# quokka-astro/quokka

Measured on AMD Instinct MI355X. Metric: Mcell-updates/s on 3D Sedov unigrid, higher is better.
Workload: dtype f64; 1 GPU; 3D Sedov blast 256x256x256 unigrid (tests/blast_unigrid_256.in scaled to 256^3 cells per GPU), 128^3 boxes, PPM+HLLC RK2, gamma=1.4, CFL 0.3, reflecting octant; cells_per_gpu=16777216, boxes_per_gpu=8, parallelism=box-decomposition x1, rk2_mode=carry, fofc_stages=0, retries=0, x_sweep_in_y_march=True

## Files before the change

### include/quokka_amd.h

```cpp
#ifndef QUOKKA_AMD_H_
#define QUOKKA_AMD_H_

#include <stdint.h>

#ifdef __cplusplus
extern "C" {
#endif

typedef struct qk_ctx qk_ctx;
typedef struct qk_level qk_level;
typedef void *qk_stream;

typedef enum qk_status {
	QK_OK = 0,
	QK_ERR_INVALID = -1,
	QK_ERR_HIP = -2,
	QK_ERR_UNSUPPORTED = -3,
	QK_ERR_STATE = -4
} qk_status;

typedef struct qk_array4 {
	double *p;
	int64_t jstride, kstride, nstride;
	int begin[3];
// ... 88 lines not shown
int qk_advect_ComputeFluxes(qk_level *lev, qk_stream s, int dir, qk_array4 *flux, const qk_array4 *left, const qk_array4 *right, double advectionVx, int nvars);
int qk_advect_PredictStep(qk_level *lev, qk_stream s, const qk_array4 *consVarOld, qk_array4 *consVarNew, const qk_array4 *const fluxArray[3], double dt,
			  const double dx[3], int nvars);
int qk_advect_AddFluxesRK2(qk_level *lev, qk_stream s, qk_array4 *U_new, const qk_array4 *U0, const qk_array4 *U1, const qk_array4 *const fluxArray[3], double dt,
			   const double dx[3], int nvars);

typedef struct qk_hydro_stage_args {
	const qk_array4 *U_in;
	const qk_array4 *U_old;
	qk_array4 *U_out;
	qk_array4 *halfFlux[3];
	qk_array4 *halfVel[3];
	qk_iarray4 *redoFlag;
	int64_t *d_redo_count;
	int *d_error_flag;
	double *d_max_signal;
	void *scratch;
	int64_t scratch_bytes;
	double dx[3];
	double dt;
	int stage;
	int reconstruction_order;
	double densityFloor, tempFloor;
	int use_dual_energy;
	double K_visc;
	int store_flux_rk2;
	qk_array4 *fluxRk2[3];
	int rk2_carry_rhs;
	qk_array4 *rhs1;
	const struct qk_carray4 *flux_mask;
	int fofc_pass;
	int prim_out;
	int prim_in;
} qk_hydro_stage_args;

int64_t qk_hydro_stage_scratch_bytes(qk_level *lev, const qk_hydro_traits *t);
int qk_hydro_stage_fused(qk_level *lev, qk_stream s, const qk_hydro_traits *t, const qk_hydro_stage_args *a);

#define QK_MAX_GROUPS 8
typedef struct qk_rad_traits {
	double c_light, c_hat, radiation_constant, Erad_floor;
	int beta_order;
	int opacity_model;
	double kappaP, kappaE, kappaF;
	int pow_mode;
	int eddington_model;
	double opacity_T_ref, opacity_T_exponent, opacity_pow_floor;
	int ngroups;
	int mg_opacity_model;
	double energy_unit;
	double rad_boundaries[QK_MAX_GROUPS + 1];
	double mg_kappa_exponent[QK_MAX_GROUPS + 1], mg_kappa_lower[QK_MAX_GROUPS + 1];
	double mg_kappa_rho_exponent, mg_kappa_T_ref, mg_kappa_T_exponent;
	int enable_dust_gas_thermal_coupling_model;
	double dust_gas_interaction_coeff;
	int thermal_model;
	double gas_dust_coupling_threshold;
	double cooling_linear_coeff[QK_MAX_GROUPS];
	double cr_heating_rate;
	int enable_photoelectric_heating;
	double pe_heating_E1_derivative;
} qk_rad_traits;

int qk_rad_ConservedToPrimitive(qk_level *lev, qk_stream s, const qk_rad_traits *rt, const qk_array4 *cons, qk_array4 *primVar, int nghost);
int qk_rad_ComputeWavespeedCorrection(qk_level *lev, qk_stream s, const qk_rad_traits *rt, const qk_hydro_traits *t, int ndim, const qk_array4 *consVar,
				      const double dx[3], qk_array4 *const eps[3]);
int qk_rad_ComputeFluxes(qk_level *lev, qk_stream s, const qk_rad_traits *rt, int dir, qk_array4 *x1Flux, const qk_array4 *x1LeftState,
			 const qk_array4 *x1RightState, const qk_array4 *consVar, const qk_array4 *wavespeed_eps);
// ... 169 lines not shown
```

### quokka_amd/capi.py

```python
from __future__ import annotations

import ctypes as C
import os

_HERE = os.path.dirname(os.path.abspath(__file__))
LIB_PATH = os.environ.get("QK_LIB_PATH", os.path.join(_HERE, "lib", "libquokka_amd.so"))

QK_OK, QK_ERR_INVALID, QK_ERR_HIP, QK_ERR_UNSUPPORTED, QK_ERR_STATE = 0, -1, -2, -3, -4
ERR_UNSUPPORTED = QK_ERR_UNSUPPORTED
HOOK_COMPILED = 100
DIR_X1, DIR_X2, DIR_X3 = 0, 1, 2
RIEMANN_HLLC, RIEMANN_LLF, RIEMANN_HLLD = 0, 1, 2
LIMITER_MINMOD, LIMITER_MC = 0, 1
BC_REFLECT_ODD, BC_INT_DIR, BC_REFLECT_EVEN, BC_FOEXTRAP, BC_EXT_DIR = -1, 0, 1, 2, 3

K_B = 1.380649e-16
M_U = 1.6605390666e-24


class Array4(C.Structure):
    _fields_ = [("p", C.c_void_p), ("jstride", C.c_int64), ("kstride", C.c_int64), ("nstride", C.c_int64),
                ("begin", C.c_int * 3), ("end", C.c_int * 3), ("ncomp", C.c_int)]


# ... 33 lines not shown
                ("ngroups", C.c_int), ("mg_opacity_model", C.c_int), ("energy_unit", C.c_double), ("rad_boundaries", C.c_double * (MAX_GROUPS + 1)),
                ("mg_kappa_exponent", C.c_double * (MAX_GROUPS + 1)), ("mg_kappa_lower", C.c_double * (MAX_GROUPS + 1)),
                ("mg_kappa_rho_exponent", C.c_double), ("mg_kappa_T_ref", C.c_double), ("mg_kappa_T_exponent", C.c_double),
                ("enable_dust_gas_thermal_coupling_model", C.c_int), ("dust_gas_interaction_coeff", C.c_double), ("thermal_model", C.c_int),
                ("gas_dust_coupling_threshold", C.c_double),
                ("cooling_linear_coeff", C.c_double * MAX_GROUPS), ("cr_heating_rate", C.c_double), ("enable_photoelectric_heating", C.c_int),
                ("pe_heating_E1_derivative", C.c_double)]

    def set_groups(self, boundaries, energy_unit, opacity_model, kappa_exponent, kappa_lower, rho_exponent=0.0, T_ref=0.0, T_exponent=0.0):
        ng = len(boundaries) - 1
        assert 2 <= ng <= MAX_GROUPS and len(kappa_exponent) == len(kappa_lower) == ng + 1
        self.ngroups, self.mg_opacity_model, self.energy_unit = ng, int(opacity_model), float(energy_unit)
        for g in range(ng + 1):
            self.rad_boundaries[g] = float(boundaries[g])
            self.mg_kappa_exponent[g] = float(kappa_exponent[g])
            self.mg_kappa_lower[g] = float(kappa_lower[g])
        self.mg_kappa_rho_exponent, self.mg_kappa_T_ref, self.mg_kappa_T_exponent = float(rho_exponent), float(T_ref), float(T_exponent)
        return self


class CloudyTables(C.Structure):
    _fields_ = [("log_nH", C.c_void_p), ("log_Tgas", C.c_void_p), ("cooling", C.c_void_p), ("heating", C.c_void_p), ("mean_mol_weight", C.c_void_p),
                ("n_nH", C.c_int), ("n_Tgas", C.c_int), ("T_min", C.c_double), ("T_max", C.c_double), ("mmw_min", C.c_double), ("mmw_max", C.c_double)]


class StageArgs(C.Structure):
    _fields_ = [("U_in", C.c_void_p), ("U_old", C.c_void_p), ("U_out", C.c_void_p),
                ("halfFlux", C.c_void_p * 3), ("halfVel", C.c_void_p * 3),
                ("redoFlag", C.c_void_p), ("d_redo_count", C.c_void_p), ("d_error_flag", C.c_void_p), ("d_max_signal", C.c_void_p),
                ("scratch", C.c_void_p), ("scratch_bytes", C.c_int64),
                ("dx", C.c_double * 3), ("dt", C.c_double), ("stage", C.c_int), ("reconstruction_order", C.c_int),
                ("densityFloor", C.c_double), ("tempFloor", C.c_double), ("use_dual_energy", C.c_int), ("K_visc", C.c_double),
                ("store_flux_rk2", C.c_int), ("fluxRk2", C.c_void_p * 3), ("rk2_carry_rhs", C.c_int), ("rhs1", C.c_void_p), ("flux_mask", C.c_void_p), ("fofc_pass", C.c_int),
                ("prim_out", C.c_int), ("prim_in", C.c_int)]


def traits(gamma=1.4, reconstruct_eint=True, ndim=3, mean_molecular_weight=M_U, boltzmann_constant=K_B,
           cs_isothermal=float("nan"), nscalars=0, nmscalars=0, eos_temperature_model=0, eos_alpha=0.0) -> HydroTraits:
    return HydroTraits(gamma, cs_isothermal, mean_molecular_weight, boltzmann_constant, int(reconstruct_eint), nscalars, nmscalars, ndim,
                       int(eos_temperature_model), float(eos_alpha))


class QkError(RuntimeError):
    pass


_lib = None


def lib() -> C.CDLL:
    global _lib
    if _lib is not None:
        return _lib
    if not os.path.exists(LIB_PATH):
        raise QkError(f"{LIB_PATH} is missing: run `python -c 'import __graft_entry__ as g; g.build()'` "
                      "(hipcc --offload-arch=gfx950). The hot path has no CPU fallback.")
    L = C.CDLL(LIB_PATH)
    vp, ci, cd = C.c_void_p, C.c_int, C.c_double
    P = C.POINTER
    L.qk_version.restype = C.c_char_p
    L.qk_last_error.restype = C.c_char_p
    L.qk_last_error.argtypes = [vp]
    L.qk_ctx_create.argtypes = [P(vp), ci]
    L.qk_ctx_destroy.argtypes = [vp]
    L.qk_level_create.argtypes = [vp, P(vp), ci, ci, P(Box)]
    L.qk_level_destroy.argtypes = [vp]
    L.qk_upload_array4_table.argtypes = [vp, ci, P(Array4), P(vp)]
    L.qk_upload_iarray4_table.argtypes = [vp, ci, P(Array4), P(vp)]
    L.qk_profile_enable.argtypes = [vp, ci]
    L.qk_profile_only.argtypes = [vp, C.c_char_p]
    L.qk_clear_bytes.argtypes = [vp, vp, vp, C.c_int64]
    L.qk_profile_reset.argtypes = [vp]
    L.qk_cloudy_tables_read.argtypes = [vp, C.c_char_p, P(CloudyTables)]
    L.qk_cloudy_tables_free.argtypes = [P(CloudyTables)]
    L.qk_cooling_tabulated.argtypes = [vp, vp, P(HydroTraits), vp, P(CloudyTables), cd, cd, vp]
    L.qk_cooling_evaluate.argtypes = [vp, vp, P(CloudyTables), cd, ci, C.c_int64, vp, vp, vp]
    L.qk_profile_num_kernels.argtypes = [vp]
    L.qk_profile_get.argtypes = [vp, ci, P(C.c_char_p), P(C.c_long), P(cd)]
    T = P(HydroTraits)
    L.qk_ReconstructStatesConstant.argtypes = [vp, vp, ci, vp, vp, vp, ci, ci]
    L.qk_ReconstructStatesPLM.argtypes = [vp, vp, ci, ci, vp, vp, vp, ci, ci]
    L.qk_ReconstructStatesPPM.argtypes = [vp, vp, ci, vp, vp, vp, ci, ci, ci, ci]
    L.qk_hydro_ConservedToPrimitive.argtypes = [vp, vp, T, vp, vp, ci]
    L.qk_hydro_ComputeFlatteningCoefficients.argtypes = [vp, vp, T, ci, vp, vp, ci]
    L.qk_hydro_FlattenShocks.argtypes = [vp, vp, T, ci, vp, vp, vp, vp, vp, vp, ci, ci]
    L.qk_hydro_ComputeFluxes.argtypes = [vp, vp, T, ci, ci, vp, vp, vp, vp, vp, cd]
    L.qk_hydro_ComputeRhsFromFluxes.argtypes = [vp, vp, T, vp, P(vp), P(cd), ci]
    L.qk_hydro_AddInternalEnergyPdV.argtypes = [vp, vp, T, vp, vp, P(cd), P(vp), vp]
    L.qk_hydro_PredictStep.argtypes = [vp, vp, T, vp, vp, vp, cd, ci, vp, vp]
    L.qk_hydro_EnforceLimits.argtypes = [vp, vp, T, cd, cd, vp]
    L.qk_hydro_SyncDualEnergy.argtypes = [vp, vp, T, vp, vp]
    L.qk_hydro_ComputeMaxSignalSpeed.argtypes = [vp, vp, T, vp, vp]
    L.qk_hydro_maxSignalSpeedLocal.argtypes = [vp, vp, T, ci, vp, vp]
    L.qk_replaceFluxes.argtypes = [vp, vp, ci, vp, vp, vp, ci]
    L.qk_Saxpy.argtypes = [vp, vp, ci, vp, cd, vp, ci]
    R = P(RadTraits)
    L.qk_rad_ConservedToPrimitive.argtypes = [vp, vp, R, vp, vp, ci]
    L.qk_rad_ComputeFluxes.argtypes = [vp, vp, R, ci, vp, vp, vp, vp, vp]
    L.qk_rad_computeRadiationFluxes.argtypes = [vp, vp, R, ci, ci, vp, P(vp), P(vp)]
    L.qk_rad_ComputeWavespeedCorrection.argtypes = [vp, vp, R, T, ci, vp, P(cd), P(vp)]
    L.qk_rad_PredictStep.argtypes = [vp, vp, R, ci, vp, vp, P(vp), cd, P(cd)]
    L.qk_rad_AddFluxesRK2.argtypes = [vp, vp, R, ci, vp, vp, vp, P(vp), P(vp), cd, P(cd)]
    L.qk_hydro_FixupState.argtypes = [vp, vp, T, cd, cd, ci, vp, vp, vp]
    L.qk_rad_stage_fused.argtypes = [vp, vp, R, ci, ci, vp, vp, vp, vp, P(vp), cd, P(cd), P(vp)]
    L.qk_rad_AddSourceTermsSingleGroup.argtypes = [vp, vp, R, T, vp, vp, cd, ci, vp, vp]
    L.qk_rad_AddSourceTermsSingleGroupMirror.argtypes = [vp, vp, R, T, vp, vp, cd, ci, vp, vp, vp]
    L.qk_rad_AddSourceTermsMultiGroup.argtypes = [vp, vp, R, T, vp, vp, cd, ci, vp, vp]
    L.qk_rad_mg_planck_fractions.argtypes = [vp, R, cd, ci, P(cd), P(cd), P(cd)]
    if hasattr(L, "qk_hydro_stage_fused"):
        L.qk_hydro_stage_scratch_bytes.argtypes = [vp, T]
        L.qk_hydro_stage_scratch_bytes.restype = C.c_int64
# ... 50 lines not shown
        L.qk_PreInterpState.argtypes = [vp, vp, vp]
        L.qk_PostInterpState.argtypes = [vp, vp, vp]
        L.qk_fluxreg_create_crse_part.argtypes = [vp, vp, P(Geometry), ci * 3, ci, P(vp)]
        L.qk_pcopy_plan_create.argtypes = [vp, P(Geometry), ci, P(Box), P(ci), ci, ci, ci, P(Box), P(ci), ci, vp, ci, ci, P(vp)]
        L.qk_pcopy_plan_destroy.argtypes = [vp]
        L.qk_pcopy_plan_num_peers.argtypes = [vp]
        L.qk_pcopy_plan_peer.argtypes = [vp, ci, P(ci), P(C.c_int64), P(C.c_int64)]
        L.qk_pcopy_plan_num_items.argtypes = [vp, ci, ci]
        L.qk_pcopy_plan_item.argtypes = [vp, ci, ci, ci, P(ci), P(ci), ci * 3, ci * 3, ci * 3, P(C.c_int64)]
        L.qk_ParallelCopy_local.argtypes = [vp, vp, vp, vp, ci, ci, ci]
        L.qk_ParallelCopy_pack.argtypes = [vp, vp, ci, vp, ci, vp]
        L.qk_ParallelCopy_unpack.argtypes = [vp, vp, ci, vp, ci, vp, ci]
    L.qk_tracer_plan_create.argtypes = [vp, P(vp), P(Geometry), cd * 3, cd * 3, cd * 3]
    L.qk_tracer_plan_destroy.argtypes = [vp]
    L.qk_tracer_plan_lattice.argtypes = [vp, ci * 3, P(C.c_int64)]
    L.qk_tracer_InitOnePerCell.argtypes = [vp, vp, cd * 3, vp * 3, vp * 3, vp, vp, C.c_int64, ci]
    L.qk_tracer_AdvectWithUmac.argtypes = [vp, vp, vp * 3, cd, C.c_int64, vp * 3, vp * 3]
    L.qk_tracer_Redistribute.argtypes = [vp, vp, C.c_int64, vp * 3, vp]
    _lib = L
    return L


BOXES_ALL, BOXES_LOCAL_ONLY, BOXES_REMOTE_DEPENDENT = 0, 1, 2
TAG_CLEAR, TAG_BUF, TAG_SET = 0, 1, 2
TAGFIELD_PRESSURE = -1

DECLARED_SYMBOLS = [
    "qk_ctx_create", "qk_ctx_destroy", "qk_last_error", "qk_version", "qk_level_create", "qk_level_destroy",
    "qk_upload_array4_table", "qk_upload_iarray4_table", "qk_clear_bytes", "qk_profile_enable", "qk_profile_only", "qk_profile_reset", "qk_profile_num_kernels", "qk_profile_get",
    "qk_ReconstructStatesConstant", "qk_ReconstructStatesPLM", "qk_ReconstructStatesPPM",
    "qk_hydro_ConservedToPrimitive", "qk_hydro_ComputeFlatteningCoefficients", "qk_hydro_FlattenShocks",
    "qk_hydro_ComputeFluxes", "qk_hydro_ComputeRhsFromFluxes", "qk_hydro_AddInternalEnergyPdV", "qk_hydro_PredictStep",
    "qk_hydro_EnforceLimits", "qk_hydro_SyncDualEnergy", "qk_hydro_ComputeMaxSignalSpeed", "qk_hydro_maxSignalSpeedLocal",
    "qk_replaceFluxes", "qk_Saxpy", "qk_hydro_FixupState", "qk_hydro_stage_scratch_bytes", "qk_hydro_stage_fused",
    "qk_rad_ConservedToPrimitive", "qk_rad_ComputeWavespeedCorrection", "qk_rad_ComputeFluxes", "qk_rad_computeRadiationFluxes", "qk_rad_PredictStep", "qk_rad_AddFluxesRK2", "qk_rad_stage_fused",
    "qk_rad_AddSourceTermsSingleGroup", "qk_rad_AddSourceTermsSingleGroupMirror", "qk_rad_AddSourceTermsMultiGroup", "qk_rad_mg_planck_fractions",
    "qk_ghost_plan_create", "qk_ghost_plan_destroy", "qk_ghost_plan_num_peers", "qk_ghost_plan_peer", "qk_ghost_plan_num_items", "qk_ghost_plan_item",
    "qk_FillBoundary_local", "qk_FillBoundary_local_int", "qk_FillBoundary_pack", "qk_FillBoundary_unpack", "qk_FillBoundary_pack_int", "qk_FillBoundary_unpack_int", "qk_SumBoundary_local", "qk_SumBoundary_pack", "qk_SumBoundary_unpack", "qk_FillPhysicalBoundary",
    "qk_FillPhysicalBoundary_subset", "qk_ghost_plan_set_components", "qk_ghost_plan_box_is_remote", "qk_ghost_plan_set_box_remote",
    "qk_tag_relative_gradient", "qk_tag_centered_gradient", "qk_avgdown_plan_create", "qk_avgdown_plan_destroy", "qk_avgdown_plan_num_items", "qk_average_down", "qk_PreInterpState", "qk_PostInterpState",
    "qk_interp_plan_create", "qk_interp_plan_destroy", "qk_interp_plan_num_items", "qk_interp_plan_item", "qk_InterpFromCoarse",
    "qk_fluxreg_create", "qk_fluxreg_destroy", "qk_fluxreg_num_items", "qk_fluxreg_item", "qk_fluxreg_reset", "qk_fluxreg_save", "qk_fluxreg_restore", "qk_fluxreg_CrseAdd", "qk_fluxreg_FineAdd",
    "qk_fluxreg_Reflux", "qk_fluxreg_set_state_component", "qk_amr_tile_flags", "qk_amr_tile_flags_periodic", "qk_amr_cluster_tiles", "qk_amr_cluster_berger_rigoutsos", "qk_copy_box",
    "qk_cloudy_tables_read", "qk_cloudy_tables_free", "qk_cooling_tabulated", "qk_cooling_evaluate",
    "qk_fluxreg_create_crse_part", "qk_pcopy_plan_create", "qk_pcopy_plan_destroy", "qk_pcopy_plan_num_peers", "qk_pcopy_plan_peer", "qk_pcopy_plan_num_items",
    "qk_pcopy_plan_item", "qk_ParallelCopy_local", "qk_ParallelCopy_pack", "qk_ParallelCopy_unpack",
    "qk_tracer_plan_create", "qk_tracer_plan_destroy", "qk_tracer_plan_lattice", "qk_tracer_InitOnePerCell", "qk_tracer_AdvectWithUmac", "qk_tracer_Redistribute",
]


def check(ctx, rc: int, what: str = "") -> None:
    if rc != QK_OK:
        msg = lib().qk_last_error(ctx).decode() if ctx else ""
        raise QkError(f"{what} failed with status {rc}: {msg}")
```

### quokka_amd/csrc/qk_hydro_fused.hip

```cpp
#include "qk_device.hpp"
#include <algorithm>
#include <cmath>
#include <cstdlib>
#include <type_traits>
#include <vector>

#include "qk_internal.hpp"

using namespace qk;

namespace
{

constexpr int NG = 4;

template <class P> QK_DEV void streamStore(P *p, double v) { __builtin_nontemporal_store(v, p); }
template <class P> QK_DEV auto streamLoad(P *p) -> double { return __builtin_nontemporal_load(p); }

struct SGeom {
	int64_t off;
	int glo[3];
	int n[3];
	int pitch;
	int64_t ncell;
// ... 831 lines not shown
	const int mrow = min(row0 + brow, hi);
	const int f = x0 + 64 * side;
	int64_t ub = Uin.idx(f - 3, mrow, ot);
	double qb[6][NV], Uc[NVAR];
#pragma unroll
	for (int m = 0; m < 6; ++m, ++ub) {
		loadPrims<NS>(Uin, ub, eos, a.reconstruct_eint, a.prim_in, qb[m], Uc);
	}
	const int64_t cb = (f - 1 - g.glo[0]) + (mrow - g.glo[1]) * st[1] + (ot - g.glo[2]) * st[2];
	const double chiL = S[cb], chiR = S[cb + 1];
	const double DyL = S[(S_AUX + 2) * T + cb], DyR = S[(S_AUX + 2) * T + cb + 1];
	const double DzL = S[(S_AUX + 3) * T + cb], DzR = S[(S_AUX + 3) * T + cb + 1];
	double qLb[NV], qRb[NV], Fb[NV], vfb;
#pragma unroll
	for (int n = 0; n < NV; ++n) {
		double unused;
		reconstructVar<ORDER>(chiL, qb[0][n], qb[1][n], qb[2][n], qb[3][n], qb[4][n], unused, qLb[n]);
		reconstructVar<ORDER>(chiR, qb[1][n], qb[2][n], qb[3][n], qb[4][n], qb[5][n], qRb[n], unused);
	}
	faceFluxAll<0, QK_RIEMANN_HLLC, false, NS>(eos, a.reconstruct_eint, 3, qLb, qRb, qb[3][PVX] - qb[2][PVX], DyL, DyR, DzL, DzR, a.K_visc, Fb, vfb);
	double(*ed)[NV + 1] = edge[brow];
	double *ef = ed[5 - side];
#pragma unroll
	for (int n = 0; n < NV; ++n) {
		ef[n] = Fb[n];
	}
	ef[NV] = vfb;
#pragma unroll
	for (int n = 0; n < NV; ++n) {
		ed[2 * side][n] = (side != 0) ? qb[3][n] : qb[1][n];
		ed[2 * side + 1][n] = (side != 0) ? qb[4][n] : qb[2][n];
	}
}
template <int DIR, int ORDER, int STAGE, bool LAST, int NS, bool CARRY, bool TWOD = false, bool FOFC = false, bool FUSEX = false>
__global__ void __launch_bounds__(64 * MARCH_BY) k_sweep_march(SweepArgs a, Eos eos)
{
	static_assert(!FUSEX || (DIR == 1 && !LAST && !TWOD && !FOFC && CARRY), "the X sweep rides on the Y sweep of a 3-D level in the carried form");
	static_assert(!(FOFC && CARRY), "the first-order flux correction pass exists for the reference's form of the RK2 average");
	static_assert(!TWOD || (DIR == 1 && LAST), "the 2-D build has one marching sweep: y, carrying the epilogue");
	constexpr int NV = NVAR + NS;
	constexpr int RHS_DIVV = S_RHS + NV;
	static_assert(DIR == 1 || DIR == 2, "marching sweeps are the strided directions");
	const BlockId blk = xcdContiguousBlock();
	const int bix = blk.x, biy = blk.y, biz = blk.z;
	const int b = biz / a.nseg;
	const int seg = biz - b * a.nseg;
	const qk_box bx = a.boxes[b];
	const SGeom g = a.geom[b];
	constexpr int OT = (DIR == 1) ? 2 : 1;
	const int i_raw = bx.lo[0] + bix * 64 + threadIdx.x;
	const int ot_raw = bx.lo[OT] + biy * MARCH_BY + threadIdx.y;
	const bool live = (i_raw <= bx.hi[0]) && (ot_raw <= bx.hi[OT]);
	const int i = min(i_raw, bx.hi[0]);
	const int ot = min(ot_raw, bx.hi[OT]);
	double sig0 = 0., sig1 = 0.;
	const int64_t T = a.total_cells;
	const int64_t st[3] = {1, g.pitch, static_cast<int64_t>(g.pitch) * g.n[1]};
	const int64_t ms = st[DIR];
	const int seglen = (bx.hi[DIR] - bx.lo[DIR] + 1 + a.nseg - 1) / a.nseg;
	const int lo = bx.lo[DIR] + seg * seglen, hi = min(lo + seglen - 1, bx.hi[DIR]);
	const int nvalid = hi - lo + 1;
	if (nvalid <= 0) {
		return;
	}
	if constexpr (FUSEX) {
		if (bx.lo[0] + bix * 64 > bx.hi[0]) {
			return;
		}
	}
	int pos[3];
	pos[0] = i;
	pos[OT] = ot;
	pos[DIR] = lo - 3;
	int64_t c = (pos[0] - g.glo[0]) * st[0] + (pos[1] - g.glo[1]) * st[1] + (pos[2] - g.glo[2]) * st[2];
	const double *S = a.scratch + g.off;
	double *Sw = a.scratch + g.off;
	RA4 Uin(a.U_in[b]);
	RA4 Uold(a.U_old[b]);
	const EpiConst ec = epiConst(eos);
	int64_t u = Uin.idx(pos[0], pos[1], pos[2]);
	const int64_t ums = (DIR == 1) ? Uin.js : Uin.ks;

	constexpr int AV = Axes<DIR, TWOD>::v, AW = Axes<DIR, TWOD>::w;
	double q[5][NV];
	double apPrev[NV], Fprev[NV];
	double vfPrev = 0., dVprev = 0., dWprev = 0.;
	bool maskCol = false;
	int maskLo = 0, maskHi = -1;
	if (CARRY && a.fluxMask != nullptr) {
		const qk_carray4 md = a.fluxMask[b];
		maskCol = live && i >= md.begin[0] && i < md.end[0] && ot >= md.begin[OT] && ot < md.end[OT];
		maskLo = md.begin[DIR];
		maskHi = md.end[DIR] - 1;
	}
	constexpr bool RING = LAST && (STAGE == 1);
	__shared__ double s_ring[RING ? 3 : 1][RING ? NV : 1][RING ? 64 * MARCH_BY : 1];
	__shared__ double s_fx[FUSEX ? MARCH_BY : 1][FUSEX ? NV + 2 : 1][FUSEX ? XW : 1];
	__shared__ double s_edge[FUSEX ? MARCH_BY : 1][FUSEX ? XROWS : 1][6][FUSEX ? NV + 1 : 1];
	double chiPrev = 1.;
	const int lself = (FUSEX && threadIdx.x == 0) ? 69 : static_cast<int>(threadIdx.x) + 2;
	const int lnext = (FUSEX && threadIdx.x == 63) ? 68 : static_cast<int>(threadIdx.x) + 3;
	const int tid = threadIdx.y * 64 + threadIdx.x;
	const bool ring = RING && a.same_old;
	int slot = 0;
	double Uo[NV];
#pragma unroll
	for (int n = 0; n < NV; ++n) {
		apPrev[n] = 0.;
		Fprev[n] = 0.;
#pragma unroll
		for (int m = 0; m < 5; ++m) {
			q[m][n] = 0.;
		}
	}

	constexpr bool PFQ = !FUSEX && NS == 0;
	double Un[NVAR];
	if constexpr (PFQ) {
#pragma unroll
		for (int n = 0; n < NVAR; ++n) {
			Un[n] = Uin.p[u + Uin.ns * n];
		}
	}
	for (int step = 0; step < nvalid + 6; ++step, c += ms, u += ums) {
#pragma unroll
		for (int n = 0; n < NV; ++n) {
			q[0][n] = q[1][n];
			q[1][n] = q[2][n];
			q[2][n] = q[3][n];
			q[3][n] = q[4][n];
		}
		{
			double Uc[NVAR];
			if constexpr (PFQ) {
#pragma unroll
				for (int n = 0; n < NVAR; ++n) {
					Uc[n] = Un[n];
					Un[n] = Uin.p[u + ums + Uin.ns * n];
				}
				primsOf<NS>(Uin, u, eos, a.reconstruct_eint, a.prim_in, Uc, q[4]);
			} else {
				loadPrims<NS>(Uin, u, eos, a.reconstruct_eint, a.prim_in, q[4], Uc);
			}
			if constexpr (RING) {
				if (ring) {
#pragma unroll
					for (int n = 0; n < NV; ++n) {
						Uo[n] = s_ring[slot][n][tid];
						s_ring[slot][n][tid] = (n < NVAR) ? Uc[n] : q[4][n];
					}
					slot = (slot == 2) ? 0 : slot + 1;
				}
			}
		}
		if (step < 4) {
			continue;
		}
		const int64_t cc = c - 2 * ms;
		const double chi = S[(S_AUX + 0) * T + cc];
		const double dV = S[(S_AUX + 1 + AV) * T + cc];
		const double dW = S[(S_AUX + 1 + AW) * T + cc];
		int fidx[3], cidx[3];
		fidx[0] = cidx[0] = i;
		fidx[OT] = cidx[OT] = ot;
		fidx[DIR] = lo + (step - 5);
		cidx[DIR] = lo + (step - 6);
		const int64_t cu = cc - ms;
		double rhs_in[NV + 1], F1[NV + 1];
		if (step >= 6) {
			if constexpr (FUSEX) {
				double(*sx)[XW] = s_fx[threadIdx.y];
				EdgeRow<NV> *edge = s_edge[threadIdx.y];
				const int rr = (step - 6) & (XROWS - 1);
				if (rr == 0) {
					fusexEdgeBatch<ORDER, NS>(a, eos, Uin, g, st, S, bx.lo[0] + bix * 64, cidx[DIR], hi, ot, edge);
					waveFence();
					stageEdgeRow<NV>(sx, edge[0]);
				}
				const double Dy = S[(S_AUX + 2) * T + cu];
				const int l = static_cast<int>(threadIdx.x) + 2;
				putColumn(sx, l, q[1]);
				waveFence();
				double amx[NV], apx[NV];
				reconstructCell<ORDER>(chiPrev, q[1], [&](int m, int n) { return sx[n][l + m]; }, amx, apx);
				const double uLeft = sx[PVX][l - 1];
				waveFence();
				putColumn(sx, l, apx);
				sx[NV][l] = Dy;
				sx[NV + 1][l] = dVprev;
				waveFence();
				double qLx[NV], Fx[NV], vfx;
				getColumn(sx, l - 1, qLx);
				const double dvl = sx[NV][l - 1], dwl = sx[NV + 1][l - 1];
				faceFluxAll<0, QK_RIEMANN_HLLC, false, NS>(eos, a.reconstruct_eint, 3, qLx, amx, q[1][PVX] - uLeft, dvl, Dy, dwl, dVprev, a.K_visc, Fx, vfx);
				waveFence();
				putColumn(sx, l, Fx);
				sx[NV][l] = vfx;
				waveFence();
#pragma unroll
				for (int n = 0; n < NV; ++n) {
					rhs_in[n] = a.inv_dx0 * (sx[n][lself] - sx[n][lnext]);
				}
				rhs_in[NV] = (sx[NV][lnext] - sx[NV][lself]) / a.dx0;
				waveFence();
				if (rr + 1 < XROWS) {
					stageEdgeRow<NV>(sx, edge[rr + 1]);
				}
			} else {
#pragma unroll
				for (int n = 0; n < NV + 1; ++n) {
					rhs_in[n] = streamLoad(&S[(S_RHS + n) * T + cu]);
				}
			}
			if (LAST && !ring && !(CARRY && STAGE == 2)) {
				const int64_t co = Uold.idx(cidx[0], cidx[1], cidx[2]);
#pragma unroll
				for (int n = 0; n < NV; ++n) {
					Uo[n] = Uold.p[co + Uold.ns * n];
				}
			}
			if (CARRY && LAST && STAGE == 2) {
				RA4 R1(a.rhs1[b]);
				const int64_t c1 = R1.idx(cidx[0], cidx[1], cidx[2]);
#pragma unroll
				for (int n = 0; n < NV + 1; ++n) {
					F1[n] = R1.p[c1 + R1.ns * n];
				}
			}
		}
		if (!CARRY && STAGE == 2 && step >= 5) {
			loadF1<NV>(a, b, fidx, F1);
		}
		double am[NV], ap[NV];
		reconstructCell<ORDER>(chi, q[2], [&](int m, int n) { return q[2 + m][n]; }, am, ap);
		if (step >= 5) {
			const double du = q[2][PVX + DIR] - q[1][PVX + DIR];
			double F[NV], vf;
			faceFluxAll<DIR, QK_RIEMANN_HLLC, TWOD, NS>(eos, a.reconstruct_eint, TWOD ? 2 : 3, apPrev, am, du, dVprev, dV, dWprev, dW, a.K_visc, F, vf);
			bool marked = false;
			if (maskCol && fidx[DIR] >= maskLo && cidx[DIR] <= maskHi) {
				CA4 M(a.fluxMask[b]);
				const int m0 = (cidx[DIR] >= maskLo) ? M(cidx[0], cidx[1], cidx[2]) : 0;
				const int m1 = (fidx[DIR] <= maskHi) ? M(fidx[0], fidx[1], fidx[2]) : 0;
				marked = (m0 | m1) != 0;
			}
			settleFace<STAGE, CARRY, FOFC, DIR, NS, TWOD>(a, eos, TWOD ? 2 : 3, b, fidx, live, marked, F1, q[1], q[2], F, vf);
			if (step >= 6) {
				double rhs[NV];
#pragma unroll
				for (int n = 0; n < NV; ++n) {
					rhs[n] = rhs_in[n] + a.inv_dx * (Fprev[n] - F[n]);
				}
				const double div_v = rhs_in[NV] + (vf - vfPrev) / a.dx;
				if (LAST) {
					if (live) {
						updateCellFrom<NS, CARRY ? STAGE : 0, FOFC, TWOD ? 2 : 3>(a, eos, ec, b, cidx[0], cidx[1], cidx[2], Uo, rhs, div_v, F1, sig0, sig1,
													    (STAGE == 1) && a.same_old && !a.reconstruct_eint && !a.prim_in, q[1][PPRES]);
					}
				} else if (live) {
#pragma unroll
					for (int n = 0; n < NV; ++n) {
						streamStore(&Sw[(S_RHS + n) * T + cu], rhs[n]);
					}
					streamStore(&Sw[RHS_DIVV * T + cu], div_v);
				}
			}
#pragma unroll
			for (int n = 0; n < NV; ++n) {
				Fprev[n] = F[n];
			}
			vfPrev = vf;
		}
#pragma unroll
		for (int n = 0; n < NV; ++n) {
			apPrev[n] = ap[n];
		}
		dVprev = dV;
		dWprev = dW;
		chiPrev = chi;
	}
	if (LAST && a.max_signal != nullptr) {
		reduceSignal(a.max_signal, sig0, sig1);
	}
}

inline auto smallLevelCells() -> int64_t
// ... 94 lines not shown
			if (cost < best) {
				best = cost;
				nseg = c;
			}
		}
	}
	return nseg;
}

auto sweepArgsFor(SweepArgs a, const qk_hydro_stage_args *args, int d) -> SweepArgs
{
	a.halfFlux = args->halfFlux[d];
	a.halfVel = args->halfVel[d];
	a.rk2Flux = args->fluxRk2[d];
	a.inv_dx = 1.0 / args->dx[d];
	a.dx = args->dx[d];
	return a;
}

auto fusexApplies(const qk_level *lev, SweepArgs const &a, bool carry, int nscalars) -> bool
{
	const char *e = std::getenv("QK_FUSEX");
	if (!carry || nscalars != 0 || lev->ndim != 3 || a.fluxMask != nullptr || (e != nullptr && std::atoi(e) == 0)) {
		return false;
	}
	for (int b = 0; b < lev->nboxes; ++b) {
		if ((lev->boxes[b].hi[0] - lev->boxes[b].lo[0] + 1) % 64 != 0) {
			return false;
		}
	}
	return true;
}

template <int ORDER, int STAGE, int NS, bool CARRY, bool FOFC = false> void launchSweeps(qk_level *lev, hipStream_t s, SweepArgs a, Eos eos, const qk_hydro_stage_args *args)
{
	const bool fusex = fusexApplies(lev, a, CARRY, NS);
	if (!fusex) {
		const SweepArgs ax = sweepArgsFor(a, args, 0);
		const int64_t slab = static_cast<int64_t>(lev->maxlen[0] + 2 * NG) * lev->maxlen[1];
		const dim3 grid(static_cast<unsigned>((slab + XOUT - 1) / XOUT), static_cast<unsigned>(lev->maxlen[2]), static_cast<unsigned>(lev->nboxes));
		ProfScope ps(lev->ctx, s, "k_sweep_x");
		if (lev->ndim == 3) {
			hipLaunchKernelGGL((k_sweep_x<ORDER, STAGE, NS, CARRY, 3, FOFC>), grid, dim3(XB), 0, s, ax, eos);
		} else if constexpr (!CARRY) {
			if (lev->ndim == 2) {
				hipLaunchKernelGGL((k_sweep_x<ORDER, STAGE, NS, false, 2, FOFC>), grid, dim3(XB), 0, s, ax, eos);
			} else {
				hipLaunchKernelGGL((k_sweep_x<ORDER, STAGE, NS, false, 1, FOFC>), grid, dim3(XB), 0, s, ax, eos);
			}
		}
	}
	if (lev->ndim == 1) {
		return;
	}
	{
		SweepArgs ay = sweepArgsFor(a, args, 1);
		ay.same_old = (lev->ndim == 2) && (args->U_in == args->U_old);
		ay.nseg = marchSegments(lev, 1, 2);
		ay.inv_dx0 = 1.0 / args->dx[0];
		ay.dx0 = args->dx[0];
		const dim3 grid((lev->maxlen[0] + 63) / 64, (lev->maxlen[2] + MARCH_BY - 1) / MARCH_BY, lev->nboxes * ay.nseg);
		ProfScope ps(lev->ctx, s, fusex ? "k_sweep_xy" : "k_sweep_y");
		if (lev->ndim == 2) {
			if constexpr (!CARRY) {
				hipLaunchKernelGGL((k_sweep_march<1, ORDER, STAGE, true, NS, false, true, FOFC>), grid, dim3(64, MARCH_BY), 0, s, ay, eos);
			}
			return;
		}
		if constexpr (CARRY && !FOFC && NS == 0) {
			if (fusex) {
				hipLaunchKernelGGL((k_sweep_march<1, ORDER, STAGE, false, NS, CARRY, false, FOFC, true>), grid, dim3(64, MARCH_BY), 0, s, ay, eos);
			}
		}
		if (!fusex) {
			hipLaunchKernelGGL((k_sweep_march<1, ORDER, STAGE, false, NS, CARRY, false, FOFC>), grid, dim3(64, MARCH_BY), 0, s, ay, eos);
		}
	}
	{
		SweepArgs az = sweepArgsFor(a, args, 2);
		az.same_old = (args->U_in == args->U_old);
		az.nseg = marchSegments(lev, 2, 1);
		const dim3 grid((lev->maxlen[0] + 63) / 64, (lev->maxlen[1] + MARCH_BY - 1) / MARCH_BY, lev->nboxes * az.nseg);
		ProfScope ps(lev->ctx, s, "k_sweep_z");
		hipLaunchKernelGGL((k_sweep_march<2, ORDER, STAGE, true, NS, CARRY, false, FOFC>), grid, dim3(64, MARCH_BY), 0, s, az, eos);
	}
}

template <int ORDER, int NS> void launchStage(qk_level *lev, hipStream_t s, SweepArgs const &a, Eos const &eos, const qk_hydro_stage_args *args)
{
	auto form = [&](auto stage) {
		constexpr int STAGE = decltype(stage)::value;
		if (args->fofc_pass != 0) {
			launchSweeps<ORDER, STAGE, NS, false, true>(lev, s, a, eos, args);
		} else if (args->rk2_carry_rhs != 0) {
			launchSweeps<ORDER, STAGE, NS, true>(lev, s, a, eos, args);
		} else {
			launchSweeps<ORDER, STAGE, NS, false>(lev, s, a, eos, args);
		}
	};
	if (args->stage == 1) {
		form(std::integral_constant<int, 1>{});
	} else {
		form(std::integral_constant<int, 2>{});
	}
}
template <int ORDER> void launchOrder(int nscalars, qk_level *lev, hipStream_t s, SweepArgs const &a, Eos const &eos, const qk_hydro_stage_args *args)
{
	switch (nscalars) {
	case 0: return launchStage<ORDER, 0>(lev, s, a, eos, args);
	case 1: return launchStage<ORDER, 1>(lev, s, a, eos, args);
	case 2: return launchStage<ORDER, 2>(lev, s, a, eos, args);
	default: return launchStage<ORDER, 3>(lev, s, a, eos, args);
	}
}

}

extern "C" {

int64_t qk_hydro_stage_scratch_bytes(qk_level *lev, const qk_hydro_traits *t)
{
	if (lev == nullptr) {
		return QK_ERR_INVALID;
	}
	if (int rc = checkTraits(lev->ctx, t); rc != QK_OK) {
		return rc;
	}
	std::vector<SGeom> g;
	const int64_t cells = scratchGeom(lev, g);
	return cells * scratchComps(t->nscalars) * static_cast<int64_t>(sizeof(double));
}

int qk_hydro_stage_fused(qk_level *lev, qk_stream stream, const qk_hydro_traits *t, const qk_hydro_stage_args *args)
{
	if (lev == nullptr) {
		return QK_ERR_INVALID;
	}
	qk_ctx *ctx = lev->ctx;
	if (int rc = checkTraits(ctx, t); rc != QK_OK) {
		return rc;
	}
	if (int rc = needsLibraryEos(ctx, t, "qk_hydro_stage_fused (EnforceLimits)"); rc != QK_OK) {
		return rc;
	}
	QK_REQUIRE(ctx, args != nullptr, "qk_hydro_stage_fused: NULL args");
	if (lev->nboxes == 0) {
		return QK_OK;
	}
	if (t->nscalars > QK_FUSED_MAX_SCALARS || t->nmscalars != 0) {
		return setError(ctx, QK_ERR_UNSUPPORTED, "qk_hydro_stage_fused: up to 3 passive scalars, no mass scalars (use the reference-shaped operators)");
	}
// ... 99 lines not shown
```

### quokka_amd/csrc/qk_internal.hpp

```cpp
#ifndef QK_INTERNAL_HPP_
#define QK_INTERNAL_HPP_

#include <hip/hip_runtime.h>

#include <cstdio>
#include <mutex>
#include <string>
#include <vector>

#include "quokka_amd.h"

struct qk_prof_pending {
	int slot;
	hipEvent_t start, stop;
};
struct qk_prof_slot {
	std::string name;
	long count = 0;
	double total_ms = 0.0;
};

struct qk_ctx {
	int device = 0;
	std::string last_error;
	std::vector<void *> owned;
	std::mutex mtx;
	bool profiling = false;
	std::string prof_only;
	std::vector<qk_prof_slot> prof_slots;
	std::vector<qk_prof_pending> prof_pending;
	std::vector<hipEvent_t> prof_free_events;
	int *counter_slots = nullptr;
};

struct qk_level {
	qk_ctx *ctx = nullptr;
	int ndim = 3;
	int nboxes = 0;
	std::vector<qk_box> boxes;
	qk_box *d_boxes = nullptr;
	int maxlen[3] = {0, 0, 0};
	void *d_sgeom = nullptr;
	int64_t sgeom_total_cells = 0;
	int *d_tile_flags = nullptr;
	size_t tile_flags_bytes = 0;
	unsigned long long *d_cooling_queue = nullptr;
};

namespace qk
{

inline auto setError(qk_ctx *ctx, int code, const char *what, const char *detail = "") -> int
{
	if (ctx != nullptr) {
		std::lock_guard<std::mutex> lock(ctx->mtx);
		ctx->last_error = std::string(what) + (detail[0] != 0 ? ": " : "") + detail;
	}
	return code;
}

#define QK_HIP_CHECK(ctx, expr)                                                                                                                      \
	do {                                                                                                                                         \
		hipError_t qk_e_ = (expr);                                                                                                           \
		if (qk_e_ != hipSuccess) {                                                                                                           \
			return qk::setError((ctx), QK_ERR_HIP, #expr, hipGetErrorString(qk_e_));                                                     \
// ... 108 lines not shown
```

### quokka_amd/simulation.py

```python
from __future__ import annotations

import ctypes as C
import math
import os
from dataclasses import dataclass
from typing import Callable, List, Optional, Sequence, Tuple

import numpy as np
import torch

from . import capi
from .hydro_system import HydroSystem, HyperbolicSystem, Saxpy, replaceFluxes
from .multifab import Context, Level, MultiFab

NGHOST_CC = 4


def chop_domain(n_cell: Sequence[int], max_grid_size: Sequence[int]) -> List[Tuple[List[int], List[int]]]:
    nb = [(n_cell[d] + max_grid_size[d] - 1) // max_grid_size[d] for d in range(3)]
    boxes = []
    for kb in range(nb[2]):
        for jb in range(nb[1]):
            for ib in range(nb[0]):
                lo, hi = [], []
# ... 528 lines not shown
        tab = (lambda mf: mf.ptr) if idx is None else (lambda mf: mf.subset_ptr(idx))
        a = capi.StageArgs()
        a.U_in, a.U_old, a.U_out = tab(U_in), tab(U_old), tab(U_out)
        nd = self.geom.ndim
        for d in range(3):
            a.halfFlux[d] = tab(self.halfFlux[d]) if d < nd else None
            a.halfVel[d] = tab(self.halfVel[d]) if d < nd else None
            a.dx[d] = self.geom.dx[d] if d < nd else 1.0
        a.redoFlag = tab(self.redoFlag)
        w = self._dev_words.data_ptr() + 32 * slot
        a.d_redo_count = C.c_void_p(w + 16)
        a.d_error_flag = C.c_void_p(w + 24)
        if self._is_final(stage):
            a.d_max_signal = C.c_void_p(w)
        sc = self.scratch if scratch is None else scratch
        a.scratch = C.c_void_p(sc.data_ptr())
        a.scratch_bytes = sc.numel() * 8
        a.dt, a.stage, a.reconstruction_order = dt, stage, self.reconstructionOrder_
        a.densityFloor, a.tempFloor, a.use_dual_energy, a.K_visc = self.densityFloor_, self.tempFloor_, self.useDualEnergy_, float(self.artificialViscosityK_)
        mask = getattr(self, "flux_mask", None)
        if self._carry_active():
            a.rk2_carry_rhs = 1
            a.rhs1 = tab(self.rhs1())
            if mask is not None:
                a.flux_mask = tab(mask)
        else:
            a.store_flux_rk2 = int(self._needs_flux_rk2())
        if a.store_flux_rk2 or a.flux_mask:
            for d in range(nd):
                a.fluxRk2[d] = tab(self.fluxRk2()[d])
        a.fofc_pass = int(fofc)
        if self._prim_now and not fofc:
            a.prim_out, a.prim_in = int(stage == 1), int(stage == 2)
        c = self.ctx
        c.check(c.L.qk_hydro_stage_fused(lev.h, c.stream(), C.byref(self.traits), C.byref(a)), "qk_hydro_stage_fused")

    def _read_words(self):
        if self.nranks > 1:
            import torch.distributed as dist
            from . import comm
            w = self._dev_words.view(2, 4)
            v = torch.cat([w[:, 0:2].reshape(-1).view(torch.float64).view(2, 2), w[:, 2:3].to(torch.float64),
                           (w[:, 3:4] & 0xFFFFFFFF).to(torch.float64)], dim=1).reshape(-1)
            comm.all_reduce(v, dist.ReduceOp.MAX)
            vals = v.tolist()
            return [vals[0:4], vals[4:8]]
        hw = self.__dict__.get("_host_words")
        if hw is None:
            hw = self.__dict__["_host_words"] = torch.zeros(8, dtype=torch.int64).pin_memory()
            self.__dict__["_host_words_np"] = hw.numpy()
        hw.copy_(self._dev_words, non_blocking=True)
        torch.cuda.current_stream(self.ctx.device).synchronize()
        a = self.__dict__["_host_words_np"]
        f = a.view(np.float64)
        return [[float(f[4 * s]), float(f[4 * s + 1]), float(a[4 * s + 2]), float(int(a[4 * s + 3]) & 0xFFFFFFFF)] for s in (0, 1)]

    def _fused_end(self, stage: int, slot: int = 0, vals=None) -> int:
        final = self._is_final(stage)
        vals = (self._read_words() if vals is None else vals)[slot]
        self._err_latched = self._err_latched or vals[3] != 0.0
        nbad = int(vals[2])
        if final and nbad == 0:
            self._signal_of_state_new = (vals[0], vals[1])
        return nbad

    def overlap_groups(self):
# ... 467 lines not shown
```

Before: 3323 Mcell-updates/s.

## Prefetch march-sweep rows into LDS with async global-to-LDS loads

Adds a prefetch variant of the marching sweep kernel for the fused XY sweep and the final Z sweep. Each wave issues global_load_lds requests for the next step's conserved-state rows, flattening/aux rows, carried RHS1 and accumulated-RHS rows into a per-wave shared-memory slot, then waits on the counters and reads from LDS. The goal is to overlap global memory latency with the current step's compute instead of loading directly from global memory. It is gated on 16-byte row alignment, box widths that are multiples of 64, no scalars and no FOFC, and an environment variable. It also adds launch counters exposed through a new C entry point.

```diff
diff --git a/include/quokka_amd.h b/include/quokka_amd.h
--- a/include/quokka_amd.h
+++ b/include/quokka_amd.h
@@ -144,8 +144,10 @@
 	int fofc_pass;
 	int prim_out;
 	int prim_in;
+	int rows_aligned16;
 } qk_hydro_stage_args;
 
+int qk_march_prefetch_counts(qk_ctx *ctx, long counts[5]);
 int64_t qk_hydro_stage_scratch_bytes(qk_level *lev, const qk_hydro_traits *t);
 int qk_hydro_stage_fused(qk_level *lev, qk_stream s, const qk_hydro_traits *t, const qk_hydro_stage_args *a);
 
diff --git a/quokka_amd/capi.py b/quokka_amd/capi.py
--- a/quokka_amd/capi.py
+++ b/quokka_amd/capi.py
@@ -89,7 +89,7 @@
                 ("dx", C.c_double * 3), ("dt", C.c_double), ("stage", C.c_int), ("reconstruction_order", C.c_int),
                 ("densityFloor", C.c_double), ("tempFloor", C.c_double), ("use_dual_energy", C.c_int), ("K_visc", C.c_double),
                 ("store_flux_rk2", C.c_int), ("fluxRk2", C.c_void_p * 3), ("rk2_carry_rhs", C.c_int), ("rhs1", C.c_void_p), ("flux_mask", C.c_void_p), ("fofc_pass", C.c_int),
-                ("prim_out", C.c_int), ("prim_in", C.c_int)]
+                ("prim_out", C.c_int), ("prim_in", C.c_int), ("rows_aligned16", C.c_int)]
 
 
 def traits(gamma=1.4, reconstruct_eint=True, ndim=3, mean_molecular_weight=M_U, boltzmann_constant=K_B,
@@ -134,6 +134,7 @@
     L.qk_cooling_evaluate.argtypes = [vp, vp, P(CloudyTables), cd, ci, C.c_int64, vp, vp, vp]
     L.qk_profile_num_kernels.argtypes = [vp]
     L.qk_profile_get.argtypes = [vp, ci, P(C.c_char_p), P(C.c_long), P(cd)]
+    L.qk_march_prefetch_counts.argtypes = [vp, P(C.c_long)]
     T = P(HydroTraits)
     L.qk_ReconstructStatesConstant.argtypes = [vp, vp, ci, vp, vp, vp, ci, ci]
     L.qk_ReconstructStatesPLM.argtypes = [vp, vp, ci, ci, vp, vp, vp, ci, ci]
@@ -250,7 +251,7 @@
     "qk_hydro_ConservedToPrimitive", "qk_hydro_ComputeFlatteningCoefficients", "qk_hydro_FlattenShocks",
     "qk_hydro_ComputeFluxes", "qk_hydro_ComputeRhsFromFluxes", "qk_hydro_AddInternalEnergyPdV", "qk_hydro_PredictStep",
     "qk_hydro_EnforceLimits", "qk_hydro_SyncDualEnergy", "qk_hydro_ComputeMaxSignalSpeed", "qk_hydro_maxSignalSpeedLocal",
-    "qk_replaceFluxes", "qk_Saxpy", "qk_hydro_FixupState", "qk_hydro_stage_scratch_bytes", "qk_hydro_stage_fused",
+    "qk_replaceFluxes", "qk_Saxpy", "qk_hydro_FixupState", "qk_hydro_stage_scratch_bytes", "qk_hydro_stage_fused", "qk_march_prefetch_counts",
     "qk_rad_ConservedToPrimitive", "qk_rad_ComputeWavespeedCorrection", "qk_rad_ComputeFluxes", "qk_rad_computeRadiationFluxes", "qk_rad_PredictStep", "qk_rad_AddFluxesRK2", "qk_rad_stage_fused",
     "qk_rad_AddSourceTermsSingleGroup", "qk_rad_AddSourceTermsSingleGroupMirror", "qk_rad_AddSourceTermsMultiGroup", "qk_rad_mg_planck_fractions",
     "qk_ghost_plan_create", "qk_ghost_plan_destroy", "qk_ghost_plan_num_peers", "qk_ghost_plan_peer", "qk_ghost_plan_num_items", "qk_ghost_plan_item",
diff --git a/quokka_amd/csrc/qk_hydro_fused.hip b/quokka_amd/csrc/qk_hydro_fused.hip
--- a/quokka_amd/csrc/qk_hydro_fused.hip
+++ b/quokka_amd/csrc/qk_hydro_fused.hip
@@ -887,10 +887,17 @@
 		ed[2 * side + 1][n] = (side != 0) ? qb[4][n] : qb[2][n];
 	}
 }
-template <int DIR, int ORDER, int STAGE, bool LAST, int NS, bool CARRY, bool TWOD = false, bool FOFC = false, bool FUSEX = false>
+using GD = const __attribute__((address_space(1))) double;
+using LD = __attribute__((address_space(3))) double;
+template <bool NT> QK_DEV void rowPair(GD *g0, int64_t laneOff, double *dst)
+{
+	__builtin_amdgcn_global_load_lds(g0 + laneOff, (LD *)dst, 16, 0, NT ? 2 : 0);
+}
+template <int DIR, int ORDER, int STAGE, bool LAST, int NS, bool CARRY, bool TWOD = false, bool FOFC = false, bool PF = false, bool FUSEX = false>
 __global__ void __launch_bounds__(64 * MARCH_BY) k_sweep_march(SweepArgs a, Eos eos)
 {
 	static_assert(!FUSEX || (DIR == 1 && !LAST && !TWOD && !FOFC && CARRY), "the X sweep rides on the Y sweep of a 3-D level in the carried form");
+	static_assert(!PF || (NS == 0 && !TWOD && !FOFC && (FUSEX || (DIR == 2 && LAST))), "the row prefetch: the fused XY sweep and the final sweep of a 3-D level");
 	static_assert(!(FOFC && CARRY), "the first-order flux correction pass exists for the reference's form of the RK2 average");
 	static_assert(!TWOD || (DIR == 1 && LAST), "the 2-D build has one marching sweep: y, carrying the epilogue");
 	constexpr int NV = NVAR + NS;
@@ -905,7 +912,7 @@
 	constexpr int OT = (DIR == 1) ? 2 : 1;
 	const int i_raw = bx.lo[0] + bix * 64 + threadIdx.x;
 	const int ot_raw = bx.lo[OT] + biy * MARCH_BY + threadIdx.y;
-	const bool live = (i_raw <= bx.hi[0]) && (ot_raw <= bx.hi[OT]);
+	const bool live = PF || ((i_raw <= bx.hi[0]) && (ot_raw <= bx.hi[OT]));
 	const int i = min(i_raw, bx.hi[0]);
 	const int ot = min(ot_raw, bx.hi[OT]);
 	double sig0 = 0., sig1 = 0.;
@@ -918,8 +925,13 @@
 	if (nvalid <= 0) {
 		return;
 	}
-	if constexpr (FUSEX) {
+	if constexpr (FUSEX || PF) {
 		if (bx.lo[0] + bix * 64 > bx.hi[0]) {
+			return;
+		}
+	}
+	if constexpr (PF) {
+		if (ot_raw > bx.hi[OT]) {
 			return;
 		}
 	}
@@ -935,6 +947,19 @@
 	const EpiConst ec = epiConst(eos);
 	int64_t u = Uin.idx(pos[0], pos[1], pos[2]);
 	const int64_t ums = (DIR == 1) ? Uin.js : Uin.ks;
+	if constexpr (PF) {
+		auto rows16 = [&](RA4 const &A) {
+			return ((((reinterpret_cast<uintptr_t>((const double *)A.p) >> 3) + static_cast<uintptr_t>(bx.lo[0] - A.bx)) | A.js | A.ks | A.ns) & 1) == 0;
+		};
+		bool ok = rows16(Uin);
+		if constexpr (CARRY && LAST && STAGE == 2) {
+			ok = ok && rows16(RA4(a.rhs1[b]));
+		}
+		if (!ok) {
+			*a.error_flag = 1;
+			return;
+		}
+	}
 
 	constexpr int AV = Axes<DIR, TWOD>::v, AW = Axes<DIR, TWOD>::w;
 	double q[5][NV];
@@ -952,8 +977,70 @@
 	__shared__ double s_ring[RING ? 3 : 1][RING ? NV : 1][RING ? 64 * MARCH_BY : 1];
 	__shared__ double s_fx[FUSEX ? MARCH_BY : 1][FUSEX ? NV + 2 : 1][FUSEX ? XW : 1];
 	__shared__ double s_edge[FUSEX ? MARCH_BY : 1][FUSEX ? XROWS : 1][6][FUSEX ? NV + 1 : 1];
+	constexpr bool R1S = CARRY && LAST && STAGE == 2;
+	constexpr int PF_R1 = NVAR + 3, PF_ACC = PF_R1 + (R1S ? NV + 1 : 0), PF_ROWS = PF_ACC + (FUSEX ? 0 : NV + 1);
+	__shared__ __attribute__((aligned(16))) double s_pf[PF ? MARCH_BY : 1][PF ? PF_ROWS * 64 : 1];
+	double *const pslot = s_pf[PF ? __builtin_amdgcn_readfirstlane(static_cast<int>(threadIdx.y)) : 0];
+	const int ptx = static_cast<int>(threadIdx.x);
+	constexpr int PF_CLO = (AV < AW) ? 1 + AV : 1 + AW, PF_CHI = (AV < AW) ? 1 + AW : 1 + AV, PF_DV = (AV < AW) ? 1 : 2, PF_DW = 3 - PF_DV;
+	qk_array4 pfR1d{};
+	if constexpr (PF && R1S) {
+		pfR1d = a.rhs1[b];
+	}
+	const RA4 pfR1(pfR1d);
+	[[maybe_unused]] GD *const pfR1p = pfR1.p;
+	[[maybe_unused]] const int64_t pfR1js = pfR1.js, pfR1ks = pfR1.ks, pfR1ns = pfR1.ns;
+	[[maybe_unused]] const int pfR1bx = pfR1.bx, pfR1by = pfR1.by, pfR1bz = pfR1.bz;
+	const int64_t pfLane = 2 * (ptx & 31);
+	const bool pfUp = (ptx & 32) != 0;
+	[[maybe_unused]] const int64_t pfOffU = pfLane + (pfUp ? Uin.ns : 0), pfOffT = pfLane + (pfUp ? T : 0), pfOffC0 = pfLane + (pfUp ? PF_CLO * T : 0),
+				       pfOffC1 = pfLane + (pfUp ? (PF_CHI - PF_CLO) * T : 0), pfOffR = pfLane + (pfUp ? pfR1d.nstride : 0);
+	[[maybe_unused]] auto pfRequest = [&](int nstep) {
+		if (nstep >= nvalid + 6) {
+			return;
+		}
+		const int x0 = bx.lo[0] + bix * 64;
+		const int otw = __builtin_amdgcn_readfirstlane(ot);
+		int pw[3];
+		pw[0] = x0;
+		pw[OT] = otw;
+		pw[DIR] = lo - 3;
+		GD *Sg = (GD *)S;
+		const int64_t cw = (pw[0] - g.glo[0]) * st[0] + (pw[1] - g.glo[1]) * st[1] + (pw[2] - g.glo[2]) * st[2];
+		const int64_t uw = Uin.idx(pw[0], pw[1], pw[2]) + nstep * ums;
+		const int64_t ccw = cw + min(max(nstep - 2, 2), nvalid + 3) * ms;
+		const int mcu = min(max(nstep - 6, 0), nvalid - 1);
+#pragma unroll
+		for (int n = 0; n < NVAR; n += 2) {
+			rowPair<false>(Uin.p + uw + Uin.ns * n, pfOffU, pslot + 64 * n);
+		}
+		rowPair<false>(Sg + S_AUX * T + ccw, pfOffC0, pslot + 64 * NVAR);
+		rowPair<false>(Sg + (S_AUX + PF_CLO) * T + ccw, pfOffC1, pslot + 64 * (NVAR + 1));
+		if constexpr (R1S) {
+			pw[DIR] = lo + mcu;
+			const int64_t r1w = (pw[0] - pfR1bx) + pfR1js * (pw[1] - pfR1by) + pfR1ks * (pw[2] - pfR1bz);
+#pragma unroll
+			for (int k = 0; k < (NV + 2) / 2; ++k) {
+				const int n = (2 * k + 1 < NV + 1) ? 2 * k : NV - 1;
+				rowPair<false>(pfR1p + r1w + pfR1ns * n, pfOffR, pslot + 64 * (PF_R1 + n));
+			}
+		}
+		if constexpr (!FUSEX) {
+#pragma unroll
+			for (int k = 0; k < (NV + 2) / 2; ++k) {
+				const int n = (2 * k + 1 < NV + 1) ? 2 * k : NV - 1;
+				rowPair<true>(Sg + (S_RHS + n) * T + cw + (3 + mcu) * ms, pfOffT, pslot + 64 * (PF_ACC + n));
+			}
+		}
+	};
+	[[maybe_unused]] auto pfNext = [&](int nstep) {
+		waveFence();
+		__builtin_amdgcn_s_waitcnt(0xC07F);
+		pfRequest(nstep);
+		waveFence();
+	};
 	double chiPrev = 1.;
-	const int lself = (FUSEX && threadIdx.x == 0) ? 69 : static_cast<int>(threadIdx.x) + 2;
+	const int lself =(FUSEX && threadIdx.x == 0) ? 69 : static_cast<int>(threadIdx.x) + 2;
 	const int lnext = (FUSEX && threadIdx.x == 63) ? 68 : static_cast<int>(threadIdx.x) + 3;
 	const int tid = threadIdx.y * 64 + threadIdx.x;
 	const bool ring = RING && a.same_old;
@@ -969,8 +1056,11 @@
 		}
 	}
 
-	constexpr bool PFQ = !FUSEX && NS == 0;
+	constexpr bool PFQ = !FUSEX && NS == 0 && !PF;
 	double Un[NVAR];
+	if constexpr (PF) {
+		pfRequest(0);
+	}
 	if constexpr (PFQ) {
 #pragma unroll
 		for (int n = 0; n < NVAR; ++n) {
@@ -978,6 +1068,7 @@
 		}
 	}
 	for (int step = 0; step < nvalid + 6; ++step, c += ms, u += ums) {
+		[[maybe_unused]] double pv[PF ? PF_ROWS - NVAR : 1];
 #pragma unroll
 		for (int n = 0; n < NV; ++n) {
 			q[0][n] = q[1][n];
@@ -987,7 +1078,23 @@
 		}
 		{
 			double Uc[NVAR];
-			if constexpr (PFQ) {
+			if constexpr (PF) {
+				if (FUSEX || step <= 6) {
+					__builtin_amdgcn_s_waitcnt(0x0F70);
+				}
+				waveFence();
+#pragma unroll
+				for (int n = 0; n < NVAR; ++n) {
+					Uc[n] = pslot[64 * n + ptx];
+				}
+				if constexpr (!FUSEX) {
+#pragma unroll
+					for (int n = 0; n < PF_ROWS - NVAR; ++n) {
+						pv[n] = pslot[64 * (NVAR + n) + ptx];
+					}
+				}
+				primsOf<NS>(Uin, u, eos, a.reconstruct_eint, a.prim_in, Uc, q[4]);
+			} else if constexpr (PFQ) {
 #pragma unroll
 				for (int n = 0; n < NVAR; ++n) {
 					Uc[n] = Un[n];
@@ -1008,13 +1115,25 @@
 				}
 			}
 		}
+		if constexpr (PF && !FUSEX) {
+			pfNext(step + 1);
+		}
 		if (step < 4) {
+			if constexpr (PF && FUSEX) {
+				pfNext(step + 1);
+			}
 			continue;
 		}
 		const int64_t cc = c - 2 * ms;
-		const double chi = S[(S_AUX + 0) * T + cc];
-		const double dV = S[(S_AUX + 1 + AV) * T + cc];
-		const double dW = S[(S_AUX + 1 + AW) * T + cc];
+		if constexpr (PF && FUSEX) {
+#pragma unroll
+			for (int n = 0; n < 3; ++n) {
+				pv[n] = pslot[64 * (NVAR + n) + ptx];
+			}
+		}
+		const double chi = PF ? pv[0] : S[(S_AUX + 0) * T + cc];
+		const double dV = PF ? pv[PF_DV] : S[(S_AUX + 1 + AV) * T + cc];
+		const double dW = PF ? pv[PF_DW] : S[(S_AUX + 1 + AW) * T + cc];
 		int fidx[3], cidx[3];
 		fidx[0] = cidx[0] = i;
 		fidx[OT] = cidx[OT] = ot;
@@ -1061,6 +1180,11 @@
 				if (rr + 1 < XROWS) {
 					stageEdgeRow<NV>(sx, edge[rr + 1]);
 				}
+			} else if constexpr (PF) {
+#pragma unroll
+				for (int n = 0; n < NV + 1; ++n) {
+					rhs_in[n] = pv[PF_ACC - NVAR + n];
+				}
 			} else {
 #pragma unroll
 				for (int n = 0; n < NV + 1; ++n) {
@@ -1074,7 +1198,12 @@
 					Uo[n] = Uold.p[co + Uold.ns * n];
 				}
 			}
-			if (CARRY && LAST && STAGE == 2) {
+			if constexpr (R1S && PF) {
+#pragma unroll
+				for (int n = 0; n < NV + 1; ++n) {
+					F1[n] = pv[PF_R1 - NVAR + n];
+				}
+			} else if (CARRY && LAST && STAGE == 2) {
 				RA4 R1(a.rhs1[b]);
 				const int64_t c1 = R1.idx(cidx[0], cidx[1], cidx[2]);
 #pragma unroll
@@ -1082,6 +1211,9 @@
 					F1[n] = R1.p[c1 + R1.ns * n];
 				}
 			}
+		}
+		if constexpr (PF && FUSEX) {
+			pfNext(step + 1);
 		}
 		if (!CARRY && STAGE == 2 && step >= 5) {
 			loadF1<NV>(a, b, fidx, F1);
@@ -1107,6 +1239,10 @@
 					rhs[n] = rhs_in[n] + a.inv_dx * (Fprev[n] - F[n]);
 				}
 				const double div_v = rhs_in[NV] + (vf - vfPrev) / a.dx;
+				if constexpr (PF && LAST) {
+					__builtin_amdgcn_s_waitcnt(0x0F70);
+					waveFence();
+				}
 				if (LAST) {
 					if (live) {
 						updateCellFrom<NS, CARRY ? STAGE : 0, FOFC, TWOD ? 2 : 3>(a, eos, ec, b, cidx[0], cidx[1], cidx[2], Uo, rhs, div_v, F1, sig0, sig1,
@@ -1267,9 +1403,36 @@
 	return true;
 }
 
+auto marchPrefetch(const qk_level *lev, const qk_hydro_stage_args *args, int nscalars, bool fofc) -> int
+{
+	const char *e = std::getenv("QK_MARCH_PREFETCH");
+	const int mode = (e != nullptr) ? std::atoi(e) : 1;
+	if (mode <= 0 || mode > 3 || args->rows_aligned16 == 0 || nscalars != 0 || lev->ndim != 3 || fofc || !rowAlign() ||
+	    (reinterpret_cast<uintptr_t>(args->scratch) & 15) != 0) {
+		return 0;
+	}
+	for (int b = 0; b < lev->nboxes; ++b) {
+		if ((lev->boxes[b].hi[0] - lev->boxes[b].lo[0] + 1) % 64 != 0) {
+			return 0;
+		}
+	}
+	return (mode == 1) ? 3 : mode - 1;
+}
+
 template <int ORDER, int STAGE, int NS, bool CARRY, bool FOFC = false> void launchSweeps(qk_level *lev, hipStream_t s, SweepArgs a, Eos eos, const qk_hydro_stage_args *args)
 {
 	const bool fusex = fusexApplies(lev, a, CARRY, NS);
+	const int pf = marchPrefetch(lev, args, NS, FOFC);
+	const bool pfxy = fusex && (pf & 1) != 0, pfz = (pf & 2) != 0;
+	if (lev->ndim == 3) {
+		std::lock_guard<std::mutex> lock(lev->ctx->mtx);
+		long *n = lev->ctx->march_prefetch_counts;
+		n[0] += pfxy ? 1 : 0;
+		n[1] += pfz ? 1 : 0;
+		n[2] += (pfz && CARRY && STAGE == 2) ? 1 : 0;
+		n[3] += pfxy ? 0 : 1;
+		n[4] += pfz ? 0 : 1;
+	}
 	if (!fusex) {
 		const SweepArgs ax = sweepArgsFor(a, args, 0);
 		const int64_t slab = static_cast<int64_t>(lev->maxlen[0] + 2 * NG) * lev->maxlen[1];
@@ -1303,8 +1466,10 @@
 			return;
 		}
 		if constexpr (CARRY && !FOFC && NS == 0) {
-			if (fusex) {
-				hipLaunchKernelGGL((k_sweep_march<1, ORDER, STAGE, false, NS, CARRY, false, FOFC, true>), grid, dim3(64, MARCH_BY), 0, s, ay, eos);
+			if (pfxy) {
+				hipLaunchKernelGGL((k_sweep_march<1, ORDER, STAGE, false, NS, CARRY, false, FOFC, true, true>), grid, dim3(64, MARCH_BY), 0, s, ay, eos);
+			} else if (fusex) {
+				hipLaunchKernelGGL((k_sweep_march<1, ORDER, STAGE, false, NS, CARRY, false, FOFC, false, true>), grid, dim3(64, MARCH_BY), 0, s, ay, eos);
 			}
 		}
 		if (!fusex) {
@@ -1317,7 +1482,14 @@
 		az.nseg = marchSegments(lev, 2, 1);
 		const dim3 grid((lev->maxlen[0] + 63) / 64, (lev->maxlen[1] + MARCH_BY - 1) / MARCH_BY, lev->nboxes * az.nseg);
 		ProfScope ps(lev->ctx, s, "k_sweep_z");
-		hipLaunchKernelGGL((k_sweep_march<2, ORDER, STAGE, true, NS, CARRY, false, FOFC>), grid, dim3(64, MARCH_BY), 0, s, az, eos);
+		if constexpr (!FOFC && NS == 0) {
+			if (pfz) {
+				hipLaunchKernelGGL((k_sweep_march<2, ORDER, STAGE, true, NS, CARRY, false, FOFC, true>), grid, dim3(64, MARCH_BY), 0, s, az, eos);
+			}
+		}
+		if (!pfz) {
+			hipLaunchKernelGGL((k_sweep_march<2, ORDER, STAGE, true, NS, CARRY, false, FOFC>), grid, dim3(64, MARCH_BY), 0, s, az, eos);
+		}
 	}
 }
 
@@ -1352,6 +1524,16 @@
 }
 
 extern "C" {
+
+int qk_march_prefetch_counts(qk_ctx *ctx, long counts[5])
+{
+	if (ctx == nullptr || counts == nullptr) {
+		return QK_ERR_INVALID;
+	}
+	std::lock_guard<std::mutex> lock(ctx->mtx);
+	std::copy(ctx->march_prefetch_counts, ctx->march_prefetch_counts + 5, counts);
+	return QK_OK;
+}
 
 int64_t qk_hydro_stage_scratch_bytes(qk_level *lev, const qk_hydro_traits *t)
 {
diff --git a/quokka_amd/csrc/qk_internal.hpp b/quokka_amd/csrc/qk_internal.hpp
--- a/quokka_amd/csrc/qk_internal.hpp
+++ b/quokka_amd/csrc/qk_internal.hpp
@@ -31,6 +31,7 @@
 	std::vector<qk_prof_pending> prof_pending;
 	std::vector<hipEvent_t> prof_free_events;
 	int *counter_slots = nullptr;
+	long march_prefetch_counts[5] = {0, 0, 0, 0, 0};
 };
 
 struct qk_level {
diff --git a/quokka_amd/simulation.py b/quokka_amd/simulation.py
--- a/quokka_amd/simulation.py
+++ b/quokka_amd/simulation.py
@@ -584,6 +584,7 @@
         a.fofc_pass = int(fofc)
         if self._prim_now and not fofc:
             a.prim_out, a.prim_in = int(stage == 1), int(stage == 2)
+        a.rows_aligned16 = int(getattr(U_in, "aligned", False) and (not a.rk2_carry_rhs or self.rhs1().aligned))
         c = self.ctx
         c.check(c.L.qk_hydro_stage_fused(lev.h, c.stream(), C.byref(self.traits), C.byref(a)), "qk_hydro_stage_fused")
 
```

Result: slower. 2954 Mcell-updates/s (-11.1%).
